# mbhall88/nohuman

Measured on AMD Instinct MI355X. Metric: Mreads/sec classified (HPRC.r2 DB, 150bp PE), higher is better.
Workload: dtype u64

## Files before the change

nohuman_amd/csrc/nh_gunzip.hip:

```cpp
#include "nh_gunzip.h"

#include <errno.h>
#include <fcntl.h>
#include <stddef.h>
#include <stdio.h>
#include <stdlib.h>
#include <string.h>
#include <sys/mman.h>
#include <sys/stat.h>
#include <unistd.h>

#include <algorithm>
#include <chrono>
#include <memory>
#include <mutex>
#include <thread>

#include "nh_inflate.h"
#include "nh_internal.h"
#include "nohuman_engine.h"

namespace nh {
namespace gz {

constexpr uint32_t WSIZE = 32768;
constexpr uint32_t MAX_MEMBERS = 4;
constexpr uint64_t NONE = ~0ull;
constexpr uint32_t NOIDX = 0xFFFFFFFFu;

enum : uint32_t {
    ST_OK = 0,
    ST_STORED = 2,
    ST_BTYPE = 3,
    ST_HEADER = 4,
    ST_ROOM = 5,
    ST_LITLEN = 6,
    ST_INPUT = 7,
    ST_DIST = 8,
    ST_MEMBERS = 9,
    ST_FAR = 10,
    ST_GZHEAD = 11,
};

struct ChunkDesc {
    uint64_t bit_start;
    uint64_t stop_bit;
    uint32_t cap;
    uint32_t pad0;
    uint64_t bit_end;
    uint32_t out_len;
    uint32_t status;
    uint32_t n_members;
    uint32_t flags;
    uint32_t blocks;
    uint32_t reach;
    uint32_t m_off[MAX_MEMBERS], m_crc[MAX_MEMBERS], m_isize[MAX_MEMBERS];
    uint32_t piece_crc[MAX_MEMBERS + 1];
    uint32_t pad2;
    uint64_t prof[12];
};

struct SegResult {
    uint64_t total;
    uint64_t end_bit;
    uint32_t n_chunks;
    uint32_t end_chunk;
    uint32_t broken;
    uint32_t bad_chunk;
    uint32_t bad_status;
    uint32_t stream_end;
    uint32_t members, pad;
    uint64_t first_start;
};

__constant__ uint16_t LBASE[29] = {3, 4, 5, 6, 7, 8, 9, 10, 11, 13, 15, 17, 19, 23, 27, 31, 35, 43, 51, 59, 67, 83, 99, 115, 131, 163, 195, 227, 258};
__constant__ uint8_t LEXT[29] = {0, 0, 0, 0, 0, 0, 0, 0, 1, 1, 1, 1, 2, 2, 2, 2, 3, 3, 3, 3, 4, 4, 4, 4, 5, 5, 5, 5, 0};
__constant__ uint16_t DBASE[30] = {1, 2, 3, 4, 5, 7, 9, 13, 17, 25, 33, 49, 65, 97, 129, 193, 257, 385, 513, 769, 1025, 1537, 2049, 3073, 4097, 6145, 8193, 12289, 16385, 24577};
__constant__ uint8_t DEXT[30] = {0, 0, 0, 0, 1, 1, 2, 2, 3, 3, 4, 4, 5, 5, 6, 6, 7, 7, 8, 8, 9, 9, 10, 10, 11, 11, 12, 12, 13, 13};
__constant__ uint8_t CLORDER[19] = {16, 17, 18, 0, 8, 7, 9, 6, 10, 5, 11, 4, 12, 3, 13, 2, 14, 1, 15};

#define LDS_ORDER() asm volatile("s_waitcnt lgkmcnt(0)" ::: "memory")

__device__ __forceinline__ uint32_t uni(uint32_t v) { return (uint32_t)__builtin_amdgcn_readfirstlane((int)v); }
__device__ __forceinline__ uint32_t rl(uint32_t v, uint32_t lane) {
    return (uint32_t)__builtin_amdgcn_readlane((int)v, (int)__builtin_amdgcn_readfirstlane((int)lane));
}
__device__ __forceinline__ uint32_t wsum(uint32_t v) {
#pragma unroll
    for (int o = 32; o > 0; o >>= 1) v += (uint32_t)__shfl_xor((int)v, o);
    return v;
}
__device__ __forceinline__ uint64_t bits_at(const uint8_t *bytes, uint64_t b) {
    struct __attribute__((packed)) U {
        uint64_t v;
    };
    return ((const U *)(bytes + (b >> 3)))->v >> (b & 7);
}

__device__ __forceinline__ uint32_t slow_symbol(uint64_t w, const uint16_t *count, const uint16_t *symlist, uint32_t &len_out) {
    uint32_t code = 0, first = 0, index = 0;
// ... 894 lines not shown
    const uint32_t per = (n + 1023) / 1024;
    unsigned long long sum = 0;
    uint32_t mine = 0;
    for (uint32_t i = 0; i < per; i++) {
        const uint32_t c = t * per + i;
        if (c < n && desc[c].bit_start != NONE) {
            sum += desc[c].out_len;
            mine++;
        }
    }
    if (mine) atomicAdd(&s_cnt, mine);
    s_scan[t] = sum;
    __syncthreads();
    for (uint32_t o = 1; o < 1024; o <<= 1) {
        const unsigned long long v = t >= o ? s_scan[t - o] : 0;
        __syncthreads();
        s_scan[t] += v;
        __syncthreads();
    }
    unsigned long long run = s_scan[t] - sum;
    for (uint32_t i = 0; i < per; i++) {
        const uint32_t c = t * per + i;
        if (c < n) {
            toff[c] = run;
            if (desc[c].bit_start != NONE) run += desc[c].out_len;
        }
    }
    if (t == 1023) res->total = s_scan[1023];
    if (t == 0) {
        res->n_chunks = s_cnt;
        res->end_chunk = last;
        res->end_bit = last != NOIDX ? desc[last].bit_end : 0;
        res->broken = s_broken;
        res->bad_chunk = s_bad;
        res->bad_status = s_bad != NOIDX ? desc[s_bad].status : 0;
        res->stream_end = stream_end ? 1u : 0u;
        res->members = s_members;
        uint64_t fs = NONE;
        for (uint32_t c = 0; c < n && fs == NONE; c++) fs = desc[c].bit_start;
        res->first_start = fs;
    }
}

constexpr uint32_t SCAN_GROUP = 32;
__device__ __forceinline__ uint16_t map_entry(const uint16_t *src, uint32_t nsym, uint32_t j) {
    if (nsym >= WSIZE) return src[nsym - WSIZE + j];
    if (j < WSIZE - nsym) return (uint16_t)(0x8000u | (j + nsym));
    return src[j - (WSIZE - nsym)];
}
__global__ __launch_bounds__(1024) void k_scan_local(const ChunkDesc *d, const uint16_t *sym, uint32_t slot_syms, uint32_t n, uint16_t *local) {
    extern __shared__ __attribute__((aligned(16))) uint8_t smem[];
    uint16_t *R = (uint16_t *)smem;
    const uint32_t g = blockIdx.x, t = threadIdx.x;
    const uint32_t c0 = g * SCAN_GROUP, c1 = c0 + SCAN_GROUP < n ? c0 + SCAN_GROUP : n;
    for (uint32_t c = c0; c < c1; c++) {
        const uint32_t nsym = d[c].bit_start == NONE ? 0u : d[c].out_len;
        const uint16_t *src = sym + (uint64_t)c * slot_syms;
        uint16_t *out = local + (size_t)c * WSIZE;
        uint16_t v[WSIZE / 1024];
#pragma unroll
        for (uint32_t k = 0; k < WSIZE / 1024; k++) {
            uint16_t x = map_entry(src, nsym, t + 1024 * k);
            if (c != c0 && (x & 0x8000u)) x = R[x & 0x7FFFu];
            v[k] = x;
        }
        __syncthreads();
#pragma unroll
        for (uint32_t k = 0; k < WSIZE / 1024; k++) {
            R[t + 1024 * k] = v[k];
            out[t + 1024 * k] = v[k];
        }
        __syncthreads();
    }
}
__global__ __launch_bounds__(1024) void k_scan_groups(const uint16_t *local, uint32_t n, uint16_t *pre) {
    extern __shared__ __attribute__((aligned(16))) uint8_t smem[];
    uint16_t *R = (uint16_t *)smem;
    const uint32_t t = threadIdx.x;
    const uint32_t ng = (n + SCAN_GROUP - 1) / SCAN_GROUP;
    for (uint32_t j = t; j < WSIZE; j += 1024) {
        R[j] = (uint16_t)(0x8000u | j);
        pre[j] = (uint16_t)(0x8000u | j);
    }
    __syncthreads();
    for (uint32_t g = 1; g < ng; g++) {
        const uint32_t last = g * SCAN_GROUP - 1;
        const uint16_t *tot = local + (size_t)last * WSIZE;
        uint16_t *out = pre + (size_t)g * WSIZE;
        uint16_t v[WSIZE / 1024];
#pragma unroll
        for (uint32_t k = 0; k < WSIZE / 1024; k++) {
            uint16_t x = tot[t + 1024 * k];
            if (x & 0x8000u) x = R[x & 0x7FFFu];
            v[k] = x;
        }
        __syncthreads();
#pragma unroll
        for (uint32_t k = 0; k < WSIZE / 1024; k++) {
            R[t + 1024 * k] = v[k];
            out[t + 1024 * k] = v[k];
        }
        __syncthreads();
    }
}
__global__ __launch_bounds__(256) void k_scan_windows(const uint16_t *local, const uint16_t *pre, const uint8_t *w0, uint8_t *windows) {
    const uint32_t c = blockIdx.x;
    uint8_t *w = windows + (size_t)c * WSIZE;
    if (c == 0) {
        for (uint32_t j = blockIdx.y * 256 + threadIdx.x; j < WSIZE; j += gridDim.y * 256) w[j] = w0[j];
        return;
    }
    const uint16_t *m = local + (size_t)(c - 1) * WSIZE;
    const uint16_t *p = pre + (size_t)((c - 1) / SCAN_GROUP) * WSIZE;
    for (uint32_t j = blockIdx.y * 256 + threadIdx.x; j < WSIZE; j += gridDim.y * 256) {
        uint16_t x = m[j];
        if (x & 0x8000u) x = p[x & 0x7FFFu];
        w[j] = x & 0x8000u ? w0[x & 0x7FFFu] : (uint8_t)x;
    }
}

__global__ __launch_bounds__(256) void k_resolve(const ChunkDesc *d, const uint16_t *sym, uint32_t slot_syms, const uint8_t *windows,
                                                 const uint64_t *toff, uint8_t *text) {
    const uint32_t c = blockIdx.x;
    if (d[c].bit_start == NONE) return;
    const uint32_t nsym = d[c].out_len;
    const uint16_t *src = sym + (uint64_t)c * slot_syms;
    const uint8_t *w = windows + (size_t)c * WSIZE;
    uint8_t *dst = text + toff[c];
    for (uint32_t i = blockIdx.y * 256 + threadIdx.x; i < nsym; i += gridDim.y * 256) {
        const uint16_t x = src[i];
        dst[i] = x & 0x8000u ? w[x & 0x7FFFu] : (uint8_t)x;
    }
}

__global__ __launch_bounds__(1024) void k_carry_window(const uint8_t *text, uint64_t total_cap, const SegResult *res, const uint8_t *old_w,
                                                       uint8_t *new_w) {
    const uint64_t total = res->total < total_cap ? res->total : total_cap;
    for (uint32_t j = threadIdx.x; j < WSIZE; j += 1024) {
        uint8_t v;
        if (total >= WSIZE) v = text[total - WSIZE + j];
        else if (j < WSIZE - total) v = old_w[j + total];
        else v = text[j - (WSIZE - total)];
        new_w[j] = v;
    }
}

constexpr uint32_t CRC_POLY = 0xEDB88320u;
__device__ __forceinline__ uint32_t multmodp(uint32_t a, uint32_t b) {
    uint32_t m = 1u << 31, p = 0;
    for (;;) {
        if (a & m) {
            p ^= b;
            if ((a & (m - 1)) == 0) break;
        }
        m >>= 1;
        b = b & 1 ? (b >> 1) ^ CRC_POLY : b >> 1;
    }
    return p;
}
__device__ __forceinline__ uint32_t x8n_modp(uint64_t n) {
    uint32_t p = 1u << 31, sq = 0x00800000u;
    while (n) {
        if (n & 1) p = multmodp(sq, p);
        sq = multmodp(sq, sq);
        n >>= 1;
    }
    return p;
}
__global__ __launch_bounds__(256) void k_crc(ChunkDesc *d, const uint64_t *toff, const uint8_t *text) {
    __shared__ uint32_t T[4][256];
    __shared__ uint32_t part[256];
    __shared__ uint32_t xl[9];
    const uint32_t c = blockIdx.x, t = threadIdx.x;
    if (d[c].bit_start == NONE) return;
    {
        uint32_t v = t;
        for (int k = 0; k < 8; k++) v = v & 1 ? (v >> 1) ^ CRC_POLY : v >> 1;
        T[0][t] = v;
    }
    __syncthreads();
    for (int k = 1; k < 4; k++) {
        const uint32_t v = T[k - 1][t];
        T[k][t] = (v >> 8) ^ T[0][v & 0xFF];
    }
    __syncthreads();
    const uint32_t nm = d[c].n_members, total = d[c].out_len;
    const uint8_t *base = text + toff[c];
    uint32_t a = 0;
    for (uint32_t p = 0; p <= nm; p++) {
        const uint32_t b = p < nm ? d[c].m_off[p] : total;
        const uint32_t len = b - a;
        uint32_t L = (len + 255) / 256;
        L = (L + 15) & ~15u;
        if (L == 0) L = 16;
        const uint32_t s0 = t * L < len ? t * L : len, s1 = (t + 1) * L < len ? (t + 1) * L : len;
        uint32_t crc = 0xFFFFFFFFu;
        const uint8_t *q = base + a + s0;
        uint32_t k = s1 - s0;
        while (k >= 16) {
            struct __attribute__((packed)) U16 {
                uint32_t v[4];
            };
            const U16 w = *(const U16 *)q;
#pragma unroll
            for (int i = 0; i < 4; i++) {
                const uint32_t x = crc ^ w.v[i];
                crc = T[3][x & 0xFF] ^ T[2][(x >> 8) & 0xFF] ^ T[1][(x >> 16) & 0xFF] ^ T[0][x >> 24];
            }
            q += 16;
            k -= 16;
        }
        while (k--) crc = (crc >> 8) ^ T[0][(crc ^ *q++) & 0xFF];
        part[t] = ~crc;
        if (t == 0) {
            uint32_t v = x8n_modp(L);
            for (int j = 0; j < 9; j++) {
                xl[j] = v;
                v = multmodp(v, v);
            }
        }
        __syncthreads();
        for (int j = 0; j < 8; j++) {
            const uint32_t w = 1u << j;
            if ((t & (2 * w - 1)) == 0) {
                const uint64_t r0 = (uint64_t)(t + w) * L, r1 = (uint64_t)(t + 2 * w) * L;
                const uint32_t rb = (uint32_t)((r1 < len ? r1 : len) - (r0 < len ? r0 : len));
                if (rb) part[t] = multmodp(rb == w * L ? xl[j] : x8n_modp(rb), part[t]) ^ part[t + w];
            }
            __syncthreads();
        }
        if (t == 0) d[c].piece_crc[p] = part[0];
        __syncthreads();
        a = b;
    }
}

}

using namespace gz;

#define GZ_TRY(x)                                                                             \
    do {                                                                                      \
        hipError_t e_ = (x);                                                                  \
        if (e_ != hipSuccess) return fail(std::string(#x) + ": " + hipGetErrorString(e_)); \
    } while (0)

namespace {
struct CacheEntry {
    int device;
    size_t bytes;
    void *p;
    bool host;
};
std::mutex g_cache_mu;
std::vector<CacheEntry> g_cache;
bool cache_on() {
    static const bool on = !(getenv("NOHUMAN_GZDEV_CACHE") && getenv("NOHUMAN_GZDEV_CACHE")[0] == '0');
    return on;
}
size_t cache_limit(bool host) {
    static const size_t dev_lim = (size_t)((getenv("NOHUMAN_GZDEV_CACHE_GB") ? atof(getenv("NOHUMAN_GZDEV_CACHE_GB")) : 64.0) * 1073741824.0);
    static const size_t host_lim = (size_t)((getenv("NOHUMAN_GZDEV_CACHE_HOST_GB") ? atof(getenv("NOHUMAN_GZDEV_CACHE_HOST_GB")) : 8.0) * 1073741824.0);
    return host ? host_lim : dev_lim;
}
void cache_release(const CacheEntry &e) {
    if (e.host) (void)hipHostFree(e.p);
    else {
        (void)dev_set(e.device);
        (void)hipFree(e.p);
    }
}
}
void dev_cache_trim() {
    std::lock_guard<std::mutex> lk(g_cache_mu);
    for (CacheEntry &e : g_cache) cache_release(e);
    g_cache.clear();
}
static size_t cache_bytes(int device, bool host) {
    std::lock_guard<std::mutex> lk(g_cache_mu);
    size_t sum = 0;
    for (const CacheEntry &e : g_cache)
        if (e.host == host && (host || device < 0 || e.device == device)) sum += e.bytes;
    return sum;
}
static void *cache_alloc(int device, size_t bytes, bool host) {
    if (!host) dev_check(device, "gzip reader, buffer allocation");
    if (cache_on() && bytes >= ((size_t)16u << 20)) {
        std::lock_guard<std::mutex> lk(g_cache_mu);
        for (size_t i = 0; i < g_cache.size(); i++) {
            CacheEntry &e = g_cache[i];
            if (e.host == host && (host || e.device == device) && e.bytes >= bytes && e.bytes <= bytes + bytes / 2) {
                void *p = e.p;
                g_cache.erase(g_cache.begin() + (long)i);
                return p;
            }
        }
    }
    void *p = nullptr;
    const hipError_t e = host ? host_malloc(&p, bytes) : dev_malloc(&p, bytes);
    if (e != hipSuccess) return nullptr;
    return p;
}
static void cache_free(int device, size_t bytes, void *p, bool host) {
    if (!p) return;
    if (cache_on() && bytes >= ((size_t)16u << 20) && bytes <= cache_limit(host)) {
        std::vector<CacheEntry> out;
        {
            std::lock_guard<std::mutex> lk(g_cache_mu);
            g_cache.push_back({device, bytes, p, host});
            size_t sum = 0;
            for (const CacheEntry &e : g_cache)
                if (e.host == host && (host || e.device == device)) sum += e.bytes;
            for (size_t i = 0; i + 1 < g_cache.size() && sum > cache_limit(host);) {
                const CacheEntry e = g_cache[i];
                if (e.host == host && (host || e.device == device)) {
                    sum -= e.bytes;
// ... 453 lines not shown
        long fake_end = -1;
        if (!spec && fake_start_ > 0 && (uint32_t)fake_start_ < n_str) {
            const uint64_t bogus = (uint64_t)fake_start_ * stretch_ * 8 + 13;
            GZA_TRY(hipMemcpyAsync(d.d_start_ + fake_start_, &bogus, 8, hipMemcpyHostToDevice, stream));
            GZA_TRY(hipStreamSynchronize(stream));
            if (getenv("NOHUMAN_GZDEV_FAKE_END")) fake_end = fake_start_;
            fake_start_ = -1;
        }
        if (spec && fake_spec_ > 0) {
            if (--fake_spec_ == 0) {
                const uint64_t bogus = 13;
                GZA_TRY(hipMemcpyAsync(d.d_start_, &bogus, 8, hipMemcpyHostToDevice, stream));
                GZA_TRY(hipStreamSynchronize(stream));
            }
        }
        hipLaunchKernelGGL(k_plan, dim3(1), dim3(1024), 0, stream, (const uint64_t *)d.d_start_, n_str, end_bit, slot_syms_, d.d_desc_);
        if (trace_) (void)hipEventRecord(d.ev_[1], stream);
        const uint32_t kflags = (j.at_eof ? 1u : 0u) | (by_headers ? 2u : 0u);
        hipLaunchKernelGGL(inflate_kernel(), dim3(n_str), dim3(64), inflate_lds(), stream, (const uint32_t *)d.d_in_, valid_bits,
                           kflags, d.d_desc_, d.d_sym_, slot_syms_, NOIDX);
        if (fake_end >= 0) hipLaunchKernelGGL(k_test_mark_end, dim3(1), dim3(1), 0, stream, d.d_desc_, (uint32_t)fake_end);
        if (trace_) (void)hipEventRecord(d.ev_[2], stream);
        uint32_t redo = 0;
        double wait_s = 0;
        for (;;) {
            hipLaunchKernelGGL(k_finish, dim3(1), dim3(1024), 0, stream, d.d_desc_, n_str, d.d_toff_, d.d_res_);
            GZA_TRY(hipMemcpyAsync(d.h_res_, d.d_res_, sizeof(SegResult), hipMemcpyDeviceToHost, stream));
            const auto w0 = std::chrono::steady_clock::now();
            GZA_TRY(hipStreamSynchronize(stream));
            wait_s += std::chrono::duration<double>(std::chrono::steady_clock::now() - w0).count();
            if (d.h_res_->bad_chunk != NOIDX && (d.h_res_->broken == NOIDX || d.h_res_->bad_chunk < d.h_res_->broken)) break;
            if (d.h_res_->broken == NOIDX) break;
            const uint32_t badc = d.h_res_->broken;
            GZA_TRY(hipMemcpyAsync(d.d_start_ + badc, &NONE, 8, hipMemcpyHostToDevice, stream));
            hipLaunchKernelGGL(k_plan, dim3(1), dim3(1024), 0, stream, (const uint64_t *)d.d_start_, n_str, end_bit, slot_syms_, d.d_desc_);
            GZA_TRY(hipMemcpyAsync(d.h_desc_, d.d_desc_, (size_t)n_str * sizeof(ChunkDesc), hipMemcpyDeviceToHost, stream));
            GZA_TRY(hipStreamSynchronize(stream));
            uint32_t prev = badc;
            while (prev > 0 && d.h_desc_[--prev].bit_start == NONE) {
            }
            if (d.h_desc_[prev].bit_start == NONE) return bad("the chunks of a piece do not chain");
            hipLaunchKernelGGL(inflate_kernel(), dim3(1), dim3(64), inflate_lds(), stream, (const uint32_t *)d.d_in_, valid_bits,
                               kflags, d.d_desc_, d.d_sym_, slot_syms_, prev);
            redo++;
            if (redo > n_str) return bad("the chunks of a piece do not chain");
        }
        j.r = *d.h_res_;
        j.redo = redo;
        {
            std::lock_guard<std::mutex> lk(st_mu_);
            st_.s_host_copy += copy_s;
            st_.s_wait += wait_s;
            st_.redecoded += redo;
            if (trace_) {
                float ms = 0;
                if (hipEventElapsedTime(&ms, d.ev_[0], d.ev_[1]) == hipSuccess) st_.ms_search += ms;
                if (hipEventElapsedTime(&ms, d.ev_[1], d.ev_[2]) == hipSuccess) st_.ms_decode += ms;
            }
        }
        j.valid = true;
        return 0;
#undef GZA_TRY
    }

    long phase_b(DevSet &d, const PieceJob &j, uint8_t *d_dst, size_t room, hipStream_t stream) {
        const SegResult &r = j.r;
        const uint32_t n_str = j.n_str;
        const uint64_t a_byte = j.a_byte;
        dev_check(d.device_, "gzip reader, phase B of a piece");
        dev_check_ptr(d_dst, d.device_, "gzip reader, phase B (text buffer)");
        dev_check_ptr(d.d_sym_, d.device_, "gzip reader, phase B (symbols)");
        if (trace_) (void)hipEventRecord(d.ev_[3], stream);
        const uint32_t gy = 4;
        if (j.by_headers) {
        } else {
            const uint32_t ng = (n_str + SCAN_GROUP - 1) / SCAN_GROUP;
            hipLaunchKernelGGL(k_scan_local, dim3(ng), dim3(1024), 2 * WSIZE, stream, (const ChunkDesc *)d.d_desc_, (const uint16_t *)d.d_sym_, slot_syms_,
                               n_str, d.d_maps_[0]);
            hipLaunchKernelGGL(k_scan_groups, dim3(1), dim3(1024), 2 * WSIZE, stream, (const uint16_t *)d.d_maps_[0], n_str, d.d_maps_[1]);
            hipLaunchKernelGGL(k_scan_windows, dim3(n_str, gy), dim3(256), 0, stream, (const uint16_t *)d.d_maps_[0], (const uint16_t *)d.d_maps_[1],
                               (const uint8_t *)d.d_win_[d.win_], d.d_windows_);
        }
        if (trace_) (void)hipEventRecord(d.ev_[4], stream);
        hipLaunchKernelGGL(k_resolve, dim3(n_str, 8), dim3(256), 0, stream, (const ChunkDesc *)d.d_desc_, (const uint16_t *)d.d_sym_, slot_syms_,
                           (const uint8_t *)d.d_windows_, (const uint64_t *)d.d_toff_, d_dst);
        if (trace_) (void)hipEventRecord(d.ev_[5], stream);
        hipLaunchKernelGGL(k_crc, dim3(n_str), dim3(256), 0, stream, d.d_desc_, (const uint64_t *)d.d_toff_, (const uint8_t *)d_dst);
        hipLaunchKernelGGL(k_carry_window, dim3(1), dim3(1024), 0, stream, (const uint8_t *)d_dst, (uint64_t)room, (const SegResult *)d.d_res_,
                           (const uint8_t *)d.d_win_[d.win_], d.d_win_[d.win_ ^ 1]);
        if (trace_) (void)hipEventRecord(d.ev_[6], stream);
        GZ_TRY(hipMemcpyAsync(d.h_desc_, d.d_desc_, (size_t)n_str * sizeof(ChunkDesc), hipMemcpyDeviceToHost, stream));
        const auto w0 = std::chrono::steady_clock::now();
        GZ_TRY(hipStreamSynchronize(stream));
        {
            std::lock_guard<std::mutex> lk(st_mu_);
            st_.s_wait += std::chrono::duration<double>(std::chrono::steady_clock::now() - w0).count();
            if (trace_) {
                float ms = 0;
                if (hipEventElapsedTime(&ms, d.ev_[3], d.ev_[4]) == hipSuccess) st_.ms_scan += ms;
                if (hipEventElapsedTime(&ms, d.ev_[4], d.ev_[5]) == hipSuccess) st_.ms_resolve += ms;
                if (hipEventElapsedTime(&ms, d.ev_[5], d.ev_[6]) == hipSuccess) st_.ms_crc += ms;
            }
        }
        d.win_ ^= 1;
        for (uint32_t c = 0; c <= r.end_chunk; c++) {
            const ChunkDesc &cd = d.h_desc_[c];
            if (cd.bit_start == NONE) continue;
#ifdef NH_GZ_PROF
            for (int i = 0; i < 12; i++) prof_[i] += cd.prof[i];
#endif
            if (cd.reach > run_len_) return fail("gzip: invalid distance too far back");
            uint32_t a = 0;
            for (uint32_t p = 0; p <= cd.n_members; p++) {
                const uint32_t b = p < cd.n_members ? cd.m_off[p] : cd.out_len;
                account(cd.piece_crc[p], b - a);
                if (p < cd.n_members && !member_end(cd.m_crc[p], cd.m_isize[p])) return -1;
                a = b;
            }
        }
        const uint64_t first_bit = pos_bit_ - 8 * a_byte;
        if (debug_)
            fprintf(stderr, "[gzdev] piece %llu: file byte %llu + bit %llu, %u stretches, %u chunks (last %u), %u decoded again, text %llu at %llu, ends at bit %llu%s%s\n",
                    (unsigned long long)st_.segments, (unsigned long long)a_byte, (unsigned long long)first_bit, n_str, r.n_chunks, r.end_chunk, j.redo,
                    (unsigned long long)r.total, (unsigned long long)st_.text_bytes, (unsigned long long)r.end_bit, r.stream_end ? " (end of stream)" : "",
                    j.first_bit == NONE ? " (decoded ahead)" : "");
        {
            std::lock_guard<std::mutex> lk(st_mu_);
            st_.segments++;
            d.pieces++;
            st_.chunks += r.n_chunks;
            st_.text_bytes += r.total;
            st_.gzip_bytes += (a_byte * 8 + r.end_bit - pos_bit_) / 8;
        }
        if (r.total) ratio_ = std::max(ratio_ * 0.9, (double)r.total / std::max<double>(1.0, (double)(r.end_bit - first_bit) / 8));
        pos_bit_ = a_byte * 8 + r.end_bit;
        if (r.stream_end) {
            if (run_len_) return fail("unexpected end of file", true);
            ended_ = true;
        } else if ((pos_bit_ >> 3) >= size_) {
            return fail("unexpected end of file", true);
        }
        return (long)r.total;
    }

    long piece(uint8_t *d_dst, size_t room, hipStream_t stream, uint64_t limit_byte = 0) {
        if (dev_set(s_->device_) != hipSuccess) return fail("hipSetDevice failed");
        const uint64_t a_byte = (pos_bit_ >> 3) / ALIGN * ALIGN;
        const uint64_t first_bit = pos_bit_ - 8 * a_byte;
        if (a_byte >= size_) return fail("unexpected end of file");
        if (host_mode_) {
            SegResult r{};
            r.bad_status = last_bad_;
            if (host_left_ == 0) {
                host_mode_ = false;
                failed_in_a_row_ = 1;
            } else {
                host_left_--;
                return host_piece(d_dst, room, stream, a_byte, first_bit, 8ull * (size_ - a_byte), r);
            }
        }
        uint32_t n = n_slots_;
        {
            const double per_stretch = ratio_ * 1.3 * (double)stretch_ + 4096;
            const uint64_t fit = (uint64_t)((double)room / per_stretch);
            if (fit < n) n = fit < 1 ? 1u : (uint32_t)fit;
        }
        for (;;) {
            PieceJob j;
            j.a_byte = a_byte;
            j.first_bit = first_bit;
// ... 371 lines not shown
        stats8[6] = s.gzip_bytes;
        stats8[7] = (uint64_t)((s.ms_search + s.ms_decode + s.ms_scan + s.ms_resolve + s.ms_crc) * 1000.0);
    }
    gz.close();
    (void)hipStreamDestroy(stream);
    (void)hipFree(d_text);
    return rc;
}

#include <atomic>
#include <condition_variable>
#include <deque>
#include <mutex>
#include <thread>

#include "nh_fastx.h"

namespace nh {
namespace fq {

constexpr uint32_t TILE = 16384;

__global__ __launch_bounds__(256) void k_nl_count(const uint8_t *text, uint64_t n, uint32_t *tile_cnt) {
    __shared__ uint32_t s_sum[4];
    const uint64_t t0 = (uint64_t)blockIdx.x * TILE;
    uint32_t c = 0;
    for (uint32_t i = threadIdx.x * 16; i < TILE; i += 256 * 16) {
        const uint64_t p = t0 + i;
        if (p + 16 <= n) {
            struct __attribute__((packed)) U16 {
                uint32_t v[4];
            };
            const U16 v = *(const U16 *)(text + p);
            const uint32_t w[4] = {v.v[0], v.v[1], v.v[2], v.v[3]};
#pragma unroll
            for (int k = 0; k < 4; k++) {
                const uint32_t x = w[k] ^ 0x0A0A0A0Au;
                c += (uint32_t)__popc(~(((x & 0x7F7F7F7Fu) + 0x7F7F7F7Fu) | x | 0x7F7F7F7Fu));
            }
        } else {
            for (uint64_t q = p; q < n && q < p + 16; q++) c += text[q] == '\n';
        }
    }
    for (int o = 32; o > 0; o >>= 1) c += (uint32_t)__shfl_xor((int)c, o);
    if ((threadIdx.x & 63) == 0) s_sum[threadIdx.x >> 6] = c;
    __syncthreads();
    if (threadIdx.x == 0) tile_cnt[blockIdx.x] = s_sum[0] + s_sum[1] + s_sum[2] + s_sum[3];
}

__global__ __launch_bounds__(1024) void k_nl_scan(uint32_t *tile_cnt, uint32_t n_tiles) {
    __shared__ unsigned long long s[1024];
    const uint32_t t = threadIdx.x, per = (n_tiles + 1023) / 1024;
    unsigned long long sum = 0;
    for (uint32_t i = 0; i < per; i++) {
        const uint32_t k = t * per + i;
        if (k < n_tiles) sum += tile_cnt[k];
    }
    s[t] = sum;
    __syncthreads();
    for (uint32_t o = 1; o < 1024; o <<= 1) {
        const unsigned long long v = t >= o ? s[t - o] : 0;
        __syncthreads();
        s[t] += v;
        __syncthreads();
    }
    unsigned long long run = s[t] - sum;
    for (uint32_t i = 0; i < per; i++) {
        const uint32_t k = t * per + i;
        if (k < n_tiles) {
            const uint32_t c = tile_cnt[k];
            tile_cnt[k] = (uint32_t)run;
            run += c;
        }
    }
    if (t == 1023) tile_cnt[n_tiles] = (uint32_t)s[1023];
}

__global__ __launch_bounds__(256) void k_nl_list(const uint8_t *text, uint64_t n, const uint32_t *tile_off, uint32_t *nl) {
    __shared__ uint32_t s_cnt[256];
    const uint64_t t0 = (uint64_t)blockIdx.x * TILE;
    const uint32_t per = TILE / 256;
    const uint64_t p0 = t0 + (uint64_t)threadIdx.x * per;
    uint64_t m = 0;
    for (uint32_t i = 0; i < per; i++)
        if (p0 + i < n && text[p0 + i] == '\n') m |= 1ull << i;
    s_cnt[threadIdx.x] = (uint32_t)__popcll(m);
    __syncthreads();
    for (uint32_t o = 1; o < 256; o <<= 1) {
        const uint32_t v = threadIdx.x >= o ? s_cnt[threadIdx.x - o] : 0;
        __syncthreads();
        s_cnt[threadIdx.x] += v;
        __syncthreads();
    }
    uint32_t at = tile_off[blockIdx.x] + s_cnt[threadIdx.x] - (uint32_t)__popcll(m);
    while (m) {
        nl[at++] = (uint32_t)(p0 + (uint64_t)__builtin_ctzll(m));
        m &= m - 1;
    }
}

__device__ __forceinline__ bool is_space(uint8_t c) { return c == ' ' || (c >= 9 && c <= 13); }

__global__ __launch_bounds__(256) void k_records(const uint8_t *text, const uint32_t *nl, uint32_t n_rec, uint32_t bf, RecRef *recs,
                                                 uint32_t *bstart, unsigned long long *bad) {
    const uint32_t r = blockIdx.x * 256 + threadIdx.x;
    if (r >= n_rec) return;
    const uint32_t l0 = 4 * r;
    const uint32_t b0 = l0 ? nl[l0 - 1] + 1 : 0, e0 = nl[l0];
    const uint32_t b1 = e0 + 1, e1 = nl[l0 + 1], b2 = e1 + 1, e2 = nl[l0 + 2], b3 = e2 + 1, e3 = nl[l0 + 3];
    uint32_t he = e0, se = e1, qe = e3;
    while (he > b0 && is_space(text[he - 1])) he--;
    while (se > b1 && is_space(text[se - 1])) se--;
    while (qe > b3 && is_space(text[qe - 1])) qe--;
    if (he == b0 || (he - b0 == 1 && text[b0] == '@')) atomicMin(bad, ((unsigned long long)r << 2) | 1ull);
    else if (text[b0] != '@') atomicMin(bad, ((unsigned long long)r << 2) | 2ull);
    uint32_t ie = b0 + 1;
    while (ie < he && text[ie] != ' ' && text[ie] != '\t' && text[ie] != '\r') ie++;
    const uint32_t rb = r / bf * bf;
    const uint32_t base = rb ? nl[4 * rb - 1] + 1 : 0;
    const bool canon = he == e0 && se == e1 && qe == e3 && e2 - b2 == 1 && text[b2] == '+';
    RecRef x;
    x.h = b0 - base;
    x.hlen = he - b0;
    x.idlen = ie > b0 ? ie - b0 - 1 : 0;
    x.s = b1 - base;
    x.slen = se - b1;
    x.q = b3 - base;
    x.qlen = qe - b3;
    x.raw_end = canon ? e3 + 1 - base : 0;
    recs[r] = x;
    if (r == rb) bstart[r / bf] = b0;
    if (r == n_rec - 1) bstart[(n_rec + bf - 1) / bf] = e3 + 1;
}

}

class DevFastqImpl {
public:
    ~DevFastqImpl() { close(); }
    int open(const char *path, const int *devices, int n_devices, std::string &err, unsigned host_threads) {
        if (!dev_gunzip_wants(path)) return 1;
        if (n_devices < 1) return 1;
        path_ = path;
        const auto t_open = std::chrono::steady_clock::now();
        lanes_.resize((size_t)n_devices);
        for (int g = 0; g < n_devices; g++) lanes_[(size_t)g].device = devices[g];
        if (nh::dev_set(devices[0]) != hipSuccess) {
            err = "hipSetDevice failed";
            return -1;
        }
        if (gz_.open(path, devices[0], 0, 0, err) != 0) return -1;
        const double t_a = std::chrono::duration<double>(std::chrono::steady_clock::now() - t_open).count();
        for (int g = 1; g < n_devices; g++)
            if (gz_.add_device(devices[g], err) != g) return -1;
        n_dev_lanes_ = lanes_.size();
        if (host_threads > 0 && gz_.ahead_ok() && !(getenv("NOHUMAN_GZ_AHEAD") && getenv("NOHUMAN_GZ_AHEAD")[0] == '0')) {
            Lane h;
            h.device = devices[0];
            h.host = true;
            lanes_.push_back(std::move(h));
            gz_.set_host_threads(host_threads);
        }
        const double t_b = std::chrono::duration<double>(std::chrono::steady_clock::now() - t_open).count();
        room_ = (size_t)3584u << 20;
        struct stat st;
        if (stat(path, &st) == 0 && (uint64_t)st.st_size * 16 + ((size_t)64u << 20) < room_) room_ = (size_t)st.st_size * 16 + ((size_t)64u << 20);
        if (const char *e = getenv("NOHUMAN_GZDEV_ROOM")) room_ = std::max<size_t>((size_t)atoll(e), (size_t)1u << 20);
        if (room_ > ((size_t)4092u << 20)) room_ = (size_t)4092u << 20;
// ... 656 lines not shown
```

Before: 1031.

## Fuse symbol resolve with per-member CRC and vectorize newline scan

```diff
diff --git a/nohuman_amd/csrc/nh_crc32.h b/nohuman_amd/csrc/nh_crc32.h
--- /dev/null
+++ b/nohuman_amd/csrc/nh_crc32.h
@@ -0,0 +1,54 @@
+#pragma once
+#include <cstdint>
+
+#if defined(__HIPCC__) || defined(__CUDACC__)
+#define NH_CRC_HD __host__ __device__
+#else
+#define NH_CRC_HD
+#endif
+
+namespace nh {
+namespace gz {
+
+constexpr uint32_t CRC_POLY = 0xEDB88320u;
+
+NH_CRC_HD constexpr uint32_t multmodp(uint32_t a, uint32_t b) {
+    uint32_t m = 1u << 31, p = 0;
+    for (;;) {
+        if (a & m) {
+            p ^= b;
+            if ((a & (m - 1)) == 0) break;
+        }
+        m >>= 1;
+        b = b & 1 ? (b >> 1) ^ CRC_POLY : b >> 1;
+    }
+    return p;
+}
+NH_CRC_HD constexpr uint32_t x8n_modp(uint64_t n) {
+    uint32_t p = 1u << 31, sq = 0x00800000u;
+    while (n) {
+        if (n & 1) p = multmodp(sq, p);
+        sq = multmodp(sq, sq);
+        n >>= 1;
+    }
+    return p;
+}
+NH_CRC_HD constexpr uint32_t mul_byte_modp(uint32_t t, uint32_t c) {
+    uint32_t p = 0;
+    for (int k = 0; k < 8; k++) {
+        if (t & (0x80u >> k)) p ^= c;
+        c = c & 1 ? (c >> 1) ^ CRC_POLY : c >> 1;
+    }
+    return p;
+}
+NH_CRC_HD constexpr uint32_t crc_table_entry(uint32_t t) {
+    for (int k = 0; k < 8; k++) t = t & 1 ? (t >> 1) ^ CRC_POLY : t >> 1;
+    return t;
+}
+
+constexpr uint32_t RS_LANES = 256, RS_BLOCK = 16;
+constexpr uint32_t RS_GAP_X = x8n_modp((RS_LANES - 1) * RS_BLOCK);
+constexpr uint32_t RS_FOLD_X[8] = {x8n_modp(16), x8n_modp(32), x8n_modp(64), x8n_modp(128), x8n_modp(256), x8n_modp(512), x8n_modp(1024), x8n_modp(2048)};
+
+}
+}
diff --git a/nohuman_amd/csrc/nh_gunzip.hip b/nohuman_amd/csrc/nh_gunzip.hip
--- a/nohuman_amd/csrc/nh_gunzip.hip
+++ b/nohuman_amd/csrc/nh_gunzip.hip
@@ -16,6 +16,7 @@
 #include <mutex>
 #include <thread>
 
+#include "nh_crc32.h"
 #include "nh_inflate.h"
 #include "nh_internal.h"
 #include "nohuman_engine.h"
@@ -1076,18 +1077,26 @@
         R[j] = (uint16_t)(0x8000u | j);
         pre[j] = (uint16_t)(0x8000u | j);
     }
+    uint16_t nx[WSIZE / 1024];
+    if (ng > 1) {
+        const uint16_t *tot = local + (size_t)(SCAN_GROUP - 1) * WSIZE;
+#pragma unroll
+        for (uint32_t k = 0; k < WSIZE / 1024; k++) nx[k] = tot[t + 1024 * k];
+    }
     __syncthreads();
     for (uint32_t g = 1; g < ng; g++) {
-        const uint32_t last = g * SCAN_GROUP - 1;
-        const uint16_t *tot = local + (size_t)last * WSIZE;
         uint16_t *out = pre + (size_t)g * WSIZE;
         uint16_t v[WSIZE / 1024];
 #pragma unroll
-        for (uint32_t k = 0; k < WSIZE / 1024; k++) {
-            uint16_t x = tot[t + 1024 * k];
-            if (x & 0x8000u) x = R[x & 0x7FFFu];
-            v[k] = x;
-        }
+        for (uint32_t k = 0; k < WSIZE / 1024; k++) v[k] = nx[k];
+        if (g + 1 < ng) {
+            const uint16_t *tot = local + (size_t)((g + 1) * SCAN_GROUP - 1) * WSIZE;
+#pragma unroll
+            for (uint32_t k = 0; k < WSIZE / 1024; k++) nx[k] = tot[t + 1024 * k];
+        }
+#pragma unroll
+        for (uint32_t k = 0; k < WSIZE / 1024; k++)
+            if (v[k] & 0x8000u) v[k] = R[v[k] & 0x7FFFu];
         __syncthreads();
 #pragma unroll
         for (uint32_t k = 0; k < WSIZE / 1024; k++) {
@@ -1113,17 +1122,117 @@
     }
 }
 
-__global__ __launch_bounds__(256) void k_resolve(const ChunkDesc *d, const uint16_t *sym, uint32_t slot_syms, const uint8_t *windows,
-                                                 const uint64_t *toff, uint8_t *text) {
-    const uint32_t c = blockIdx.x;
+constexpr uint32_t RS_GY = MAX_MEMBERS + 1;
+struct __attribute__((packed)) U16B {
+    uint32_t v[4];
+};
+template <bool WIN>
+__global__ __launch_bounds__(256) void k_resolve_crc(ChunkDesc *d, const uint16_t *sym, uint32_t slot_syms, const uint8_t *windows,
+                                                     const uint64_t *toff, uint8_t *text) {
+    __shared__ __attribute__((aligned(16))) uint8_t win[WIN ? WSIZE : 16];
+    __shared__ uint32_t T[4][256], Z[4][256];
+    __shared__ uint32_t part[256];
+    const uint32_t c = blockIdx.x, t = threadIdx.x;
     if (d[c].bit_start == NONE) return;
     const uint32_t nsym = d[c].out_len;
+    const uint32_t nm = d[c].n_members, y = blockIdx.y;
+    if (y > nm) return;
+    const uint32_t i0 = y ? d[c].m_off[y - 1] : 0;
+    uint32_t i1 = y < nm ? d[c].m_off[y] : nsym;
+    if (i1 > nsym) i1 = nsym;
+    if (i0 >= i1) {
+        if (t == 0) d[c].piece_crc[y] = 0;
+        return;
+    }
+    T[0][t] = crc_table_entry(t);
+    Z[3][t] = mul_byte_modp(t, RS_GAP_X);
+    if (WIN) {
+        const uint4 *ws = (const uint4 *)(windows + (size_t)c * WSIZE);
+        uint4 *wl = (uint4 *)win;
+        for (uint32_t j = t; j < WSIZE / 16; j += 256) wl[j] = ws[j];
+    }
+    __syncthreads();
+    for (int k = 1; k < 4; k++) {
+        const uint32_t v = T[k - 1][t], z = Z[4 - k][t];
+        T[k][t] = (v >> 8) ^ T[0][v & 0xFF];
+        Z[3 - k][t] = (z >> 8) ^ T[0][z & 0xFF];
+    }
+    __syncthreads();
     const uint16_t *src = sym + (uint64_t)c * slot_syms;
-    const uint8_t *w = windows + (size_t)c * WSIZE;
     uint8_t *dst = text + toff[c];
-    for (uint32_t i = blockIdx.y * 256 + threadIdx.x; i < nsym; i += gridDim.y * 256) {
-        const uint16_t x = src[i];
-        dst[i] = x & 0x8000u ? w[x & 0x7FFFu] : (uint8_t)x;
+    auto one = [&](uint32_t x) -> uint32_t { return WIN && (x & 0x8000u) ? win[x & 0x7FFFu] : x & 0xFFu; };
+    const uint32_t A = (uint32_t)((uintptr_t)dst & 15);
+    const uint32_t P0 = i0 + A, P1 = i1 + A;
+    const uint32_t Pa = (P0 + 15) & ~15u, Pb = P1 & ~15u;
+    const uint32_t nb = Pb > Pa ? (Pb - Pa) >> 4 : 0;
+    const uint32_t head_end = Pa < P1 ? Pa : P1;
+    uint32_t s = 0;
+    if (t == 0) {
+        s = 0xFFFFFFFFu;
+        for (uint32_t p = P0; p < head_end; p++) {
+            const uint32_t b = one(src[p - A]);
+            dst[p - A] = (uint8_t)b;
+            s = (s >> 8) ^ T[0][(s ^ b) & 0xFF];
+        }
+    }
+    if (nb) {
+        uint32_t k = t;
+        U16B ca = {}, cb = {};
+        if (k < nb) {
+            const uint16_t *q = src + (Pa - A) + 16 * k;
+            ca = *(const U16B *)q;
+            cb = *(const U16B *)(q + 8);
+        }
+        bool first = true;
+        while (k < nb) {
+            const uint32_t kn = k + 256;
+            U16B na = ca, nbv = cb;
+            if (kn < nb) {
+                const uint16_t *q = src + (Pa - A) + 16 * kn;
+                na = *(const U16B *)q;
+                nbv = *(const U16B *)(q + 8);
+            }
+            const uint32_t sw[8] = {ca.v[0], ca.v[1], ca.v[2], ca.v[3], cb.v[0], cb.v[1], cb.v[2], cb.v[3]};
+            uint32_t o[4];
+            if (WIN && ((sw[0] | sw[1] | sw[2] | sw[3] | sw[4] | sw[5] | sw[6] | sw[7]) & 0x80008000u)) {
+#pragma unroll
+                for (int j = 0; j < 4; j++)
+                    o[j] = one(sw[2 * j] & 0xFFFFu) | (one(sw[2 * j] >> 16) << 8) | (one(sw[2 * j + 1] & 0xFFFFu) << 16) | (one(sw[2 * j + 1] >> 16) << 24);
+            } else {
+#pragma unroll
+                for (int j = 0; j < 4; j++)
+                    o[j] = (sw[2 * j] & 0xFFu) | ((sw[2 * j] >> 8) & 0xFF00u) | ((sw[2 * j + 1] & 0xFFu) << 16) | ((sw[2 * j + 1] << 8) & 0xFF000000u);
+            }
+            *(uint4 *)(dst + (Pa - A) + 16 * k) = make_uint4(o[0], o[1], o[2], o[3]);
+            if (!first) s = Z[0][s & 0xFF] ^ Z[1][(s >> 8) & 0xFF] ^ Z[2][(s >> 16) & 0xFF] ^ Z[3][s >> 24];
+#pragma unroll
+            for (int j = 0; j < 4; j++) {
+                const uint32_t x = s ^ o[j];
+                s = T[3][x & 0xFF] ^ T[2][(x >> 8) & 0xFF] ^ T[1][(x >> 16) & 0xFF] ^ T[0][x >> 24];
+            }
+            first = false;
+            k = kn;
+            ca = na;
+            cb = nbv;
+        }
+        const uint32_t r = nb - ((nb - 1) & ~255u);
+        part[(t - r) & 255] = s;
+        __syncthreads();
+#pragma unroll
+        for (int j = 0; j < 8; j++) {
+            const uint32_t w = 1u << j;
+            if ((t & (2 * w - 1)) == 0) part[t] = multmodp(RS_FOLD_X[j], part[t]) ^ part[t + w];
+            __syncthreads();
+        }
+        s = part[0];
+    }
+    if (t == 0) {
+        for (uint32_t p = Pb > head_end ? Pb : head_end; p < P1; p++) {
+            const uint32_t b = one(src[p - A]);
+            dst[p - A] = (uint8_t)b;
+            s = (s >> 8) ^ T[0][(s ^ b) & 0xFF];
+        }
+        d[c].piece_crc[y] = ~s;
     }
 }
 
@@ -1136,96 +1245,6 @@
         else if (j < WSIZE - total) v = old_w[j + total];
         else v = text[j - (WSIZE - total)];
         new_w[j] = v;
-    }
-}
-
-constexpr uint32_t CRC_POLY = 0xEDB88320u;
-__device__ __forceinline__ uint32_t multmodp(uint32_t a, uint32_t b) {
-    uint32_t m = 1u << 31, p = 0;
-    for (;;) {
-        if (a & m) {
-            p ^= b;
-            if ((a & (m - 1)) == 0) break;
-        }
-        m >>= 1;
-        b = b & 1 ? (b >> 1) ^ CRC_POLY : b >> 1;
-    }
-    return p;
-}
-__device__ __forceinline__ uint32_t x8n_modp(uint64_t n) {
-    uint32_t p = 1u << 31, sq = 0x00800000u;
-    while (n) {
-        if (n & 1) p = multmodp(sq, p);
-        sq = multmodp(sq, sq);
-        n >>= 1;
-    }
-    return p;
-}
-__global__ __launch_bounds__(256) void k_crc(ChunkDesc *d, const uint64_t *toff, const uint8_t *text) {
-    __shared__ uint32_t T[4][256];
-    __shared__ uint32_t part[256];
-    __shared__ uint32_t xl[9];
-    const uint32_t c = blockIdx.x, t = threadIdx.x;
-    if (d[c].bit_start == NONE) return;
-    {
-        uint32_t v = t;
-        for (int k = 0; k < 8; k++) v = v & 1 ? (v >> 1) ^ CRC_POLY : v >> 1;
-        T[0][t] = v;
-    }
-    __syncthreads();
-    for (int k = 1; k < 4; k++) {
-        const uint32_t v = T[k - 1][t];
-        T[k][t] = (v >> 8) ^ T[0][v & 0xFF];
-    }
-    __syncthreads();
-    const uint32_t nm = d[c].n_members, total = d[c].out_len;
-    const uint8_t *base = text + toff[c];
-    uint32_t a = 0;
-    for (uint32_t p = 0; p <= nm; p++) {
-        const uint32_t b = p < nm ? d[c].m_off[p] : total;
-        const uint32_t len = b - a;
-        uint32_t L = (len + 255) / 256;
-        L = (L + 15) & ~15u;
-        if (L == 0) L = 16;
-        const uint32_t s0 = t * L < len ? t * L : len, s1 = (t + 1) * L < len ? (t + 1) * L : len;
-        uint32_t crc = 0xFFFFFFFFu;
-        const uint8_t *q = base + a + s0;
-        uint32_t k = s1 - s0;
-        while (k >= 16) {
-            struct __attribute__((packed)) U16 {
-                uint32_t v[4];
-            };
-            const U16 w = *(const U16 *)q;
-#pragma unroll
-            for (int i = 0; i < 4; i++) {
-                const uint32_t x = crc ^ w.v[i];
-                crc = T[3][x & 0xFF] ^ T[2][(x >> 8) & 0xFF] ^ T[1][(x >> 16) & 0xFF] ^ T[0][x >> 24];
-            }
-            q += 16;
-            k -= 16;
-        }
-        while (k--) crc = (crc >> 8) ^ T[0][(crc ^ *q++) & 0xFF];
-        part[t] = ~crc;
-        if (t == 0) {
-            uint32_t v = x8n_modp(L);
-            for (int j = 0; j < 9; j++) {
-                xl[j] = v;
-                v = multmodp(v, v);
-            }
-        }
-        __syncthreads();
-        for (int j = 0; j < 8; j++) {
-            const uint32_t w = 1u << j;
-            if ((t & (2 * w - 1)) == 0) {
-                const uint64_t r0 = (uint64_t)(t + w) * L, r1 = (uint64_t)(t + 2 * w) * L;
-                const uint32_t rb = (uint32_t)((r1 < len ? r1 : len) - (r0 < len ? r0 : len));
-                if (rb) part[t] = multmodp(rb == w * L ? xl[j] : x8n_modp(rb), part[t]) ^ part[t + w];
-            }
-            __syncthreads();
-        }
-        if (t == 0) d[c].piece_crc[p] = part[0];
-        __syncthreads();
-        a = b;
     }
 }
 
@@ -1845,10 +1864,13 @@
                                (const uint8_t *)d.d_win_[d.win_], d.d_windows_);
         }
         if (trace_) (void)hipEventRecord(d.ev_[4], stream);
-        hipLaunchKernelGGL(k_resolve, dim3(n_str, 8), dim3(256), 0, stream, (const ChunkDesc *)d.d_desc_, (const uint16_t *)d.d_sym_, slot_syms_,
-                           (const uint8_t *)d.d_windows_, (const uint64_t *)d.d_toff_, d_dst);
+        if (j.by_headers)
+            hipLaunchKernelGGL(k_resolve_crc<false>, dim3(n_str, RS_GY), dim3(256), 0, stream, d.d_desc_, (const uint16_t *)d.d_sym_, slot_syms_,
+                               (const uint8_t *)d.d_windows_, (const uint64_t *)d.d_toff_, d_dst);
+        else
+            hipLaunchKernelGGL(k_resolve_crc<true>, dim3(n_str, RS_GY), dim3(256), 0, stream, d.d_desc_, (const uint16_t *)d.d_sym_, slot_syms_,
+                               (const uint8_t *)d.d_windows_, (const uint64_t *)d.d_toff_, d_dst);
         if (trace_) (void)hipEventRecord(d.ev_[5], stream);
-        hipLaunchKernelGGL(k_crc, dim3(n_str), dim3(256), 0, stream, d.d_desc_, (const uint64_t *)d.d_toff_, (const uint8_t *)d_dst);
         hipLaunchKernelGGL(k_carry_window, dim3(1), dim3(1024), 0, stream, (const uint8_t *)d_dst, (uint64_t)room, (const SegResult *)d.d_res_,
                            (const uint8_t *)d.d_win_[d.win_], d.d_win_[d.win_ ^ 1]);
         if (trace_) (void)hipEventRecord(d.ev_[6], stream);
@@ -2386,8 +2408,22 @@
     const uint32_t per = TILE / 256;
     const uint64_t p0 = t0 + (uint64_t)threadIdx.x * per;
     uint64_t m = 0;
-    for (uint32_t i = 0; i < per; i++)
-        if (p0 + i < n && text[p0 + i] == '\n') m |= 1ull << i;
+    if (p0 + per <= n) {
+        struct __attribute__((packed)) U16 {
+            uint32_t v[4];
+        };
+        const U16 *q = (const U16 *)(text + p0);
+        const U16 a[4] = {q[0], q[1], q[2], q[3]};
+#pragma unroll
+        for (int k = 0; k < 16; k++) {
+            const uint32_t x = a[k >> 2].v[k & 3] ^ 0x0A0A0A0Au;
+            const uint32_t z = ~(((x & 0x7F7F7F7Fu) + 0x7F7F7F7Fu) | x | 0x7F7F7F7Fu) >> 7;
+            m |= (uint64_t)((z | z >> 7 | z >> 14 | z >> 21) & 0xFu) << (4 * k);
+        }
+    } else {
+        for (uint32_t i = 0; i < per; i++)
+            if (p0 + i < n && text[p0 + i] == '\n') m |= 1ull << i;
+    }
     s_cnt[threadIdx.x] = (uint32_t)__popcll(m);
     __syncthreads();
     for (uint32_t o = 1; o < 256; o <<= 1) {
```

Measured after the change: 1043 (median of 2 runs). About the same (+1.2%).
